# YuliangXiu/ICON

Measured on NVIDIA H100. Metric: M query-points/sec at 256^3 grid, higher is better.
Workload: dtype f32

## Files before the change

icon_b200/_C.py:

```python
import ctypes
import os

_HERE = os.path.dirname(os.path.abspath(__file__))
LIB_PATH = os.environ.get("ICON_B200_LIB") or os.path.join(_HERE, "libicon_b200.so")

if not os.path.exists(LIB_PATH):
    raise ImportError(
        f"{LIB_PATH} is missing: the CUDA extension must be built (python -m icon_b200.build); "
        "icon_b200 has no CPU or PyTorch fallback.")

lib = ctypes.CDLL(LIB_PATH)

_vp, _i, _i64, _f, _sz = ctypes.c_void_p, ctypes.c_int, ctypes.c_int64, ctypes.c_float, ctypes.c_size_t

_SIGS = {
    "icon_version": (_i, []),
    "icon_last_error": (ctypes.c_char_p, []),
    "icon_launch_count": (_i64, []),
    "icon_profile_enable": (_i, [_i]),
    "icon_profile_last_query": (_i, [_vp]),
    "icon_smpl_workspace_bytes": (_sz, [_i, _i]),
    "icon_smpl_prepare": (_i, [_vp, _vp, _vp, _vp, _i, _i, _vp, _sz, _vp]),
    "icon_query_workspace_bytes": (_sz, [_i64, _i, _i]),
    "icon_set_mlp_impl": (_i, [_i]),
    "icon_get_mlp_impl": (_i, []),
    "icon_query": (_i, [_i, _vp, _i64, _i64, _i64, _vp, _vp, _i, _i, _i, _vp, _i, _vp, _i, _i, _vp, _vp, _i, _f,
                        _vp, _vp, _sz, _vp]),
    "icon_query_feats": (_i, [_i, _vp, _i64, _i64, _i64, _vp, _vp, _i, _i, _i, _vp, _i, _vp, _i, _i, _vp, _vp, _i, _f,
                              _i, _vp, _vp, _sz, _vp]),
    "icon_set_sdf_policy": (_i, [_i, _i64, _i64]),
    "icon_set_sdf_bricks": (_i, [_i, _i64]),
    "icon_sdf_brick_info": (_i, [_vp, _i, _i, _vp]),
    "icon_sdf_only": (_i, [_vp, _i64, _i64, _i64, _vp, _vp, _i, _i, _vp, _vp, _vp, _sz, _vp]),
    "icon_sdf_bruteforce": (_i, [_vp, _i64, _i64, _i64, _vp, _vp, _i, _i, _vp, _vp, _vp]),
    "icon_mesh_workspace_bytes": (_sz, [_i, _i]),
    "icon_mesh_prepare": (_i, [_vp, _vp, _i, _i, _vp, _sz, _vp]),
    "icon_mesh_distance": (_i, [_vp, _i64, _vp, _i, _i, _vp, _vp, _vp]),
    "icon_mesh_sample_workspace_bytes": (_sz, [_i]),
    "icon_mesh_sample": (_i, [_vp, _vp, _i, _i, _vp, _i, ctypes.c_uint64, _vp, _vp, _vp, _vp, _sz, _vp]),
    "icon_mlp_only": (_i, [_vp, _i, _i64, _vp, _vp, _vp, _vp]),
    "icon_display": (_i, [_vp, _i, _vp, _vp]),
    "icon_grid_upsample": (_i, [_vp, _vp, _i, _f, _vp, _vp, _vp, _vp]),
    "icon_grid_dilate": (_i, [_vp, _i, _i, _vp, _vp, _vp]),
    "icon_compact_workspace_bytes": (_sz, [_i]),
    "icon_grid_compact": (_i, [_vp, _vp, _i, _i, _vp, _vp, _vp, _vp, _i64, _vp, _vp, _sz, _vp]),
    "icon_grid_scatter": (_i, [_vp, _vp, _vp, _i64, _vp]),
    "icon_grid_init_points": (_i, [_i, _i, _vp, _vp, _vp, _vp]),
    "icon_grid_count_above": (_i, [_vp, _i64, _f, _vp, _vp]),
    "icon_conv_nhwc_workspace_bytes": (_sz, [_i, _i, _i, _i, _i]),
    "icon_conv_nhwc": (_i, [_vp, _vp, _vp, _vp, _vp, _i, _vp, _vp, _vp, _i, _i, _i, _i, _i, _i, _i, _i, _i, _i, _i, _i, _i,
                           _i, _vp, _i, _i, _i, _vp, _vp, _sz, _vp]),
    "icon_norm_finalize": (_i, [_vp, _vp, _vp, _vp, _i, _i, _i, ctypes.c_double, _f, _vp]),
    "icon_act_nhwc": (_i, [_vp, _i, _i, _vp, _vp, _vp, _vp, _i, _f, _vp, _vp, _vp, _vp, _i, _i, _i, _i, _i, _i, _i, _i, _vp]),
    "icon_splitk_instnorm_act": (_i, [_vp, _i, _vp, _vp, _vp, _vp, _vp, _i, _i, _i, _i, _i, _i, _i, _f, _vp]),
    "icon_col2im7": (_i, [_vp, _vp, _vp, _i, _i, _i, _i, _i, _i, _vp]),
    "icon_ew_nhwc": (_i, [_i, _vp, _vp, _vp, _vp, _vp, _i, _i, _i, _i, _vp]),
    "icon_nchw_to_nhwc": (_i, [_vp, _vp, _vp, _i, _i, _i64, _vp]),
    "icon_nhwc_to_nchw": (_i, [_vp, _vp, _i, _i, _i, _i, _i64, _vp]),
# ... 107 lines not shown
```

icon_b200/build.py:

```python
import os
import subprocess
import sys
from concurrent.futures import ThreadPoolExecutor

HERE = os.path.dirname(os.path.abspath(__file__))
CSRC = os.path.join(HERE, "csrc")
OBJ = os.path.join(HERE, "build")
LIB = os.path.join(HERE, "libicon_b200.so")

ARCH = ["-gencode", "arch=compute_90a,code=sm_90a"]
COMMON = ["-O3", "-std=c++17", "-lineinfo", "-Xcompiler", "-fPIC", "-Xcompiler", "-Wall",
          "--expt-relaxed-constexpr"]
SOURCES = {
    "common.cu": [],
    "smpl.cu": ["-fmad=false"],
    "sdf.cu": ["-fmad=false"],
    "mlp.cu": [],
    "mlp_tc.cu": [],
    "engine.cu": [],
    "conv.cu": [],
    "conv_nhwc.cu": [],
    "act_nhwc.cu": [],
    "mc.cu": [],
    "clean.cu": [],
# ... 19 lines not shown
    return out


def gen_tables():
    from . import mc_tables as T
    path = os.path.join(CSRC, "mc_tables.inc")
    lines = ["// GENERATED by icon_b200/build.py from icon_b200/mc_tables.py -- do not edit.",
             "__constant__ unsigned char c_num_verts[256] = {" + ",".join(str(v) for v in T.NUM_VERTS) + "};",
             "__constant__ signed char c_tri_table[256][16] = {"]
    for row in T.TRI_TABLE:
        lines.append("  {" + ",".join(str(v) for v in row) + "},")
    lines.append("};")
    lines.append("__constant__ signed char c_edge_owner[12][4] = {")
    for row in _edge_owner():
        lines.append("  {" + ",".join(str(v) for v in row) + "},")
    lines.append("};")
    text = "\n".join(lines) + "\n"
    if not os.path.exists(path) or open(path).read() != text:
        with open(path, "w") as f:
            f.write(text)
    return path


def _newest_header():
    t = 0.0
    for root, _, files in os.walk(CSRC):
        for f in files:
            if f.endswith((".cuh", ".inc", ".h")):
                t = max(t, os.path.getmtime(os.path.join(root, f)))
    t = max(t, os.path.getmtime(os.path.join(os.path.dirname(HERE), "include", "icon_b200.h")))
    return t


def build(force=False, verbose=False):
    os.makedirs(OBJ, exist_ok=True)
    gen_tables()
    hdr_t = _newest_header()
    jobs = []
    for src, extra in SOURCES.items():
        s = os.path.join(CSRC, src)
        o = os.path.join(OBJ, src.replace(".cu", ".o"))
        if force or not os.path.exists(o) or os.path.getmtime(o) < max(os.path.getmtime(s), hdr_t):
            cmd = ["nvcc", "-c", s, "-o", o] + ARCH + COMMON + extra
            if verbose:
                cmd += ["-Xptxas", "-v"]
            jobs.append(cmd)

    def run(cmd):
        r = subprocess.run(cmd, stdout=subprocess.PIPE, stderr=subprocess.STDOUT, text=True)
        return cmd, r.returncode, r.stdout

    with ThreadPoolExecutor(max_workers=6) as ex:
        for cmd, rc, out in ex.map(run, jobs):
            if verbose or rc:
                print(" ".join(cmd))
                print(out)
            if rc:
                raise RuntimeError("nvcc failed for " + cmd[2])
    objs = [os.path.join(OBJ, s.replace(".cu", ".o")) for s in SOURCES]
    if jobs or force or not os.path.exists(LIB):
        cmd = ["nvcc", "-shared", "-o", LIB] + objs + ARCH + ["-lcudart"]
        subprocess.check_call(cmd)
    return LIB


if __name__ == "__main__":
    print(build(force="--force" in sys.argv, verbose="--verbose" in sys.argv))
```

icon_b200/csrc/mlp_tc.cu:

```cuda
#include <cuda_fp16.h>

#include "common.cuh"
#include "query_common.cuh"
#include "wgmma.cuh"

namespace icon {

constexpr int TC_THREADS = 384;
constexpr int TC_M = 128;
constexpr int NSTAGE = 4;
constexpr int STAGE_BYTES = 32768;
constexpr int STAGES_PER_TILE = 20;
static_assert(STAGES_PER_TILE % NSTAGE == 0 && NSTAGE % 2 == 0, "layer-1 hi / lo pairs must stay on stages (2i, 2i + 1)");
constexpr int GATHER_THREADS = 96;

constexpr int TCB_W0 = 0;
constexpr int TCB_W1 = 32768;
constexpr int TCB_W2 = TCB_W1 + 8 * 65536;
constexpr int TCB_W2T = TCB_W2 + 4 * 32768;
constexpr int TCB_F32 = TCB_W2T + 8192;
constexpr int TCB_F32_FLOATS = 512 + 256 + 128 + 144 + 4;
constexpr int TCB_BYTES = TCB_F32 + TCB_F32_FLOATS * 4;
static_assert(TCB_BYTES == ICON_MLP_TC_BYTES, "blob layout");

constexpr int SM_STAGE = 0;
constexpr int SM_W0 = NSTAGE * STAGE_BYTES;
constexpr int SM_X0 = SM_W0 + 32768;
constexpr int X0_H = 0;
constexpr int X0_L = 4096;
constexpr int X0_F = 8192;
constexpr int X0_SLOT = 16384;
constexpr int SM_F32 = SM_X0 + 2 * X0_SLOT;
constexpr int SM_W2T = (SM_F32 + TCB_F32_FLOATS * 4 + 127) / 128 * 128;
constexpr int SM_BAR = SM_W2T + 8192;
constexpr int NBAR = 2 * NSTAGE + 5;
constexpr int SM_TOTAL = SM_BAR + NBAR * 8;
constexpr int TC_SMEM_BYTES = SM_TOTAL + 1024;
static_assert(TC_SMEM_BYTES <= 227 * 1024, "shared memory");

enum { B_FULL0 = 0, B_EMPTY0 = NSTAGE, B_W0RDY = 2 * NSTAGE, B_XFULL0 = 2 * NSTAGE + 1, B_XEMPTY0 = 2 * NSTAGE + 3 };

constexpr int REG_CONSUMER = 224, REG_PRODUCER = 56;
static_assert(2 * 128 * REG_CONSUMER + 128 * REG_PRODUCER <= 168 * TC_THREADS, "register split");

__device__ __forceinline__ void act_frag64(const float *d, const float *bias, uint32_t (&ah)[4][4], uint32_t (&al)[4][4]) {
#pragma unroll
    for (int kk = 0; kk < 4; ++kk) {
// ... 56 lines not shown
                        if (ch < d) xf[ch * TC_M] = bilinear(q.feat + (size_t)(fb + ch) * q.H * q.W, q.H, q.W, xyz.x, xyz.y);
                }
            } else if (MODE == 1) {
                if (q.C == 12) {
#pragma unroll
                    for (int ch = 0; ch < 12; ++ch)
                        xf[ch * TC_M] = bilinear(q.feat + (size_t)ch * q.H * q.W, q.H, q.W, xyz.x, xyz.y);
                } else {
#pragma unroll
                    for (int ch = 0; ch < 14; ++ch)
                        if (ch < q.C) xf[ch * TC_M] = bilinear(q.feat + (size_t)ch * q.H * q.W, q.H, q.W, xyz.x, xyz.y);
                }
                if (q.C < 15) xf[q.C * TC_M] = xyz.z;
            } else {
                const size_t vs = (size_t)q.VD * q.VD * q.VD;
                if (q.C == 6) {
#pragma unroll
                    for (int ch = 0; ch < 6; ++ch)
                        xf[ch * TC_M] = bilinear(q.feat + (size_t)ch * q.H * q.W, q.H, q.W, xyz.x, xyz.y);
                } else {
#pragma unroll
                    for (int ch = 0; ch < 8; ++ch)
                        if (ch < q.C) xf[ch * TC_M] = bilinear(q.feat + (size_t)ch * q.H * q.W, q.H, q.W, xyz.x, xyz.y);
                }
#pragma unroll
                for (int ch = 0; ch < 7; ++ch)
                    if (q.C + ch < 15) xf[(q.C + ch) * TC_M] = trilinear(q.vol + ch * vs, q.VD, xyz.x, xyz.y, xyz.z);
            }
        }
    }
    xf[15 * TC_M] = in_cube;
}

template <int MODE>
__global__ void __launch_bounds__(TC_THREADS, 1) k_query_mlp_tc(QueryParams q, const uint8_t *__restrict__ blob) {
    using namespace wg;
    extern __shared__ uint8_t smem_raw[];
    const uint32_t raw = s32(smem_raw);
    const uint32_t base = (raw + 1023u) & ~1023u;
    uint8_t *sm = smem_raw + (base - raw);
    const float *sf32 = reinterpret_cast<const float *>(sm + SM_F32);
    const float *sb1 = sf32 + 512, *sw3 = sf32 + 896, *sb3 = sf32 + 1040;
    const uint32_t bar0 = base + SM_BAR;
    auto BAR = [&](int i) { return bar0 + 8u * (uint32_t)i; };

    const int tid = threadIdx.x, warp = tid >> 5, lane = tid & 31;
    const int64_t ntiles = (q.N + TC_M - 1) / TC_M;

    if (tid == 0) {
        for (int s = 0; s < NSTAGE; ++s) { mbar_init(BAR(B_FULL0 + s), 1); mbar_init(BAR(B_EMPTY0 + s), 8); }
        mbar_init(BAR(B_W0RDY), 1);
        for (int b = 0; b < 2; ++b) { mbar_init(BAR(B_XFULL0 + b), GATHER_THREADS); mbar_init(BAR(B_XEMPTY0 + b), 8); }
        asm volatile("fence.mbarrier_init.release.cluster;" ::: "memory");
    }
    __syncthreads();

    if (warp >= 8) {
        asm volatile("setmaxnreg.dec.sync.aligned.u32 %0;" ::"n"(REG_PRODUCER));
        if (warp == 8) {
            if (lane == 0) {
                mbar_expect_tx(BAR(B_W0RDY), 32768 + TCB_F32_FLOATS * 4 + 8192);
                bulk_g2s(base + SM_W0, blob + TCB_W0, 32768, BAR(B_W0RDY));
                bulk_g2s(base + SM_F32, blob + TCB_F32, TCB_F32_FLOATS * 4, BAR(B_W0RDY));
                bulk_g2s(base + SM_W2T, blob + TCB_W2T, 8192, BAR(B_W0RDY));
                uint32_t cnt = 0;
                for (int64_t tile = blockIdx.x; tile < ntiles; tile += gridDim.x) {
                    for (int i = 0; i < STAGES_PER_TILE; ++i, ++cnt) {
                        const uint32_t s = cnt % NSTAGE, ph = (cnt / NSTAGE) & 1;
                        mbar_wait(BAR(B_EMPTY0 + s), ph ^ 1);
                        const uint32_t dst = base + SM_STAGE + s * STAGE_BYTES, full = BAR(B_FULL0 + s);
                        mbar_expect_tx(full, STAGE_BYTES);
                        const uint8_t *src = i < 16 ? blob + TCB_W1 + (size_t)i * 32768 : blob + TCB_W2 + (size_t)(i - 16) * 32768;
                        bulk_g2s(dst, src, STAGE_BYTES, full);
                    }
                }
            }
        } else {
            const int gt = tid - 9 * 32;
            for (uint32_t it = 0; blockIdx.x + (int64_t)it * gridDim.x < ntiles; ++it) {
                const int b = it & 1;
                mbar_wait(BAR(B_XEMPTY0 + b), ((it >> 1) & 1) ^ 1);
                uint8_t *xs = sm + SM_X0 + b * X0_SLOT;
                for (int r = gt; r < TC_M; r += GATHER_THREADS) {
                    float *xf = reinterpret_cast<float *>(xs + X0_F) + r;
                    gather_point<MODE>(q, (blockIdx.x + (int64_t)it * gridDim.x) * TC_M + r, xf);
                    uint32_t hi[8], lo[8];
#pragma unroll
                    for (int i = 0; i < 7; ++i) split2(xf[2 * i * TC_M], xf[(2 * i + 1) * TC_M], hi[i], lo[i]);
                    split2(xf[14 * TC_M], 1.f, hi[7], lo[7]);
                    const int off = (r >> 3) * 128 + (r & 7) * 16;
                    *reinterpret_cast<uint4 *>(xs + X0_H + off) = make_uint4(hi[0], hi[1], hi[2], hi[3]);
                    *reinterpret_cast<uint4 *>(xs + X0_H + off + 2048) = make_uint4(hi[4], hi[5], hi[6], hi[7]);
                    *reinterpret_cast<uint4 *>(xs + X0_L + off) = make_uint4(lo[0], lo[1], lo[2], lo[3]);
                    *reinterpret_cast<uint4 *>(xs + X0_L + off + 2048) = make_uint4(lo[4], lo[5], lo[6], lo[7]);
                }
                fence_proxy_async();
                mbar_arrive(BAR(B_XFULL0 + b));
            }
        }
        return;
    }

    asm volatile("setmaxnreg.inc.sync.aligned.u32 %0;" ::"n"(REG_CONSUMER));
    const int g = warp >> 2;
    const int rf = 64 * g + 16 * (warp & 3) + (lane >> 2);
    const int cq = 2 * (lane & 3);
    uint32_t cnt = 0;
    auto stage_wait = [&](uint32_t c) {
        const uint32_t s = c % NSTAGE;
        mbar_wait(BAR(B_FULL0 + s), (c / NSTAGE) & 1);
        return s;
    };
    auto warp_arrive = [&](int bar) {
        __syncwarp();
        if (lane == 0) mbar_arrive(BAR(bar));
    };
    const uint64_t dw2th = desc_nosw(base + SM_W2T, 2048, 128), dw2tl = desc_nosw(base + SM_W2T + 4096, 2048, 128);
    mbar_wait(BAR(B_W0RDY), 0);

    uint32_t it = 0;
    for (int64_t tile = blockIdx.x; tile < ntiles; tile += gridDim.x, ++it) {
        const int b = it & 1;
        const uint32_t xs = base + SM_X0 + b * X0_SLOT;
        const uint64_t dx0h = desc_nosw(xs + X0_H + g * 1024, 2048, 128), dx0l = desc_nosw(xs + X0_L + g * 1024, 2048, 128);
        mbar_wait(BAR(B_XFULL0 + b), (it >> 1) & 1);

        auto layer0 = [&](int j, float (&a0)[32]) {
            const uint64_t w0h = desc_nosw(base + SM_W0 + j * 1024, 8192, 128), w0l = w0h + (16384 >> 4);
            fence();
            mma_ss<64>(a0, dx0h, w0h, 0);
            mma_ss<64>(a0, dx0h, w0l, 1);
            mma_ss<64>(a0, dx0l, w0h, 1);
            commit();
        };
        float acc1[128];
        auto layer1 = [&](int j, uint32_t (&ch)[4][4], uint32_t (&cl)[4][4], uint32_t (&nh)[4][4], uint32_t (&nl)[4][4]) {
            wait<0>();
            if (j) { warp_arrive(B_EMPTY0 + (cnt - 2) % NSTAGE); warp_arrive(B_EMPTY0 + (cnt - 1) % NSTAGE); }
            float a0[32];
            if (j < 7) layer0(j + 1, a0);
            const uint32_t s = stage_wait(cnt);
            stage_wait(cnt + 1);
            const uint64_t bh = desc_sw128(base + SM_STAGE + s * STAGE_BYTES), bl = bh + (STAGE_BYTES >> 4);
            fence();
#pragma unroll
            for (int kk = 0; kk < 4; ++kk) {
                mma_rs<256>(acc1, ch[kk], bh + 2 * kk, (j | kk) != 0);
                mma_rs<256>(acc1, ch[kk], bl + 2 * kk, 1);
                mma_rs<256>(acc1, cl[kk], bh + 2 * kk, 1);
            }
            commit();
            cnt += 2;
            if (j < 7) {
                wait<1>();
                fence_regs(a0);
                act_frag64(a0, nullptr, nh, nl);
            }
        };
        uint32_t xh[4][4], xl[4][4], yh[4][4], yl[4][4];
        {
            float a0[32];
            layer0(0, a0);
            wait<0>();
            fence_regs(a0);
            act_frag64(a0, nullptr, xh, xl);
        }
#pragma unroll
        for (int j = 0; j < 8; j += 2) {
            layer1(j, xh, xl, yh, yl);
            layer1(j + 1, yh, yl, xh, xl);
        }
        wait<0>();
        fence_regs(acc1);
        warp_arrive(B_EMPTY0 + (cnt - 2) % NSTAGE);
        warp_arrive(B_EMPTY0 + (cnt - 1) % NSTAGE);

        float acc2[64];
        auto layer2 = [&](int c, uint32_t (&ch)[4][4], uint32_t (&cl)[4][4]) {
            const uint32_t s = stage_wait(cnt);
            const uint64_t bh = desc_sw128(base + SM_STAGE + s * STAGE_BYTES), bl = bh + (16384 >> 4);
            fence();
#pragma unroll
            for (int kk = 0; kk < 4; ++kk) {
                mma_rs<128>(acc2, ch[kk], bh + 2 * kk, (c | kk) != 0);
                mma_rs<128>(acc2, ch[kk], bl + 2 * kk, 1);
                mma_rs<128>(acc2, cl[kk], bh + 2 * kk, 1);
            }
            commit();
            ++cnt;
            if (c) {
                wait<1>();
                warp_arrive(B_EMPTY0 + (cnt - 2) % NSTAGE);
            }
        };
        act_frag64(acc1, sb1 + cq, xh, xl);
        layer2(0, xh, xl);
        act_frag64(acc1 + 32, sb1 + 64 + cq, yh, yl);
        layer2(1, yh, yl);
        act_frag64(acc1 + 64, sb1 + 128 + cq, xh, xl);
        layer2(2, xh, xl);
        act_frag64(acc1 + 96, sb1 + 192 + cq, yh, yl);
        layer2(3, yh, yl);
        fence();
        mma_ss<128>(acc2, dx0h, dw2th, 1);
        mma_ss<128>(acc2, dx0h, dw2tl, 1);
        mma_ss<128>(acc2, dx0l, dw2th, 1);
        commit();
        wait<0>();
        fence_regs(acc2);
        warp_arrive(B_EMPTY0 + (cnt - 1) % NSTAGE);

        const float *x0f = reinterpret_cast<const float *>(sm + (xs - base) + X0_F);
        float s0 = 0.f, s1 = 0.f;
#pragma unroll
        for (int i = 0; i < 16; ++i) {
            const float w0 = sw3[8 * i + cq], w1 = sw3[8 * i + cq + 1];
            float v0 = acc2[4 * i], v1 = acc2[4 * i + 1], v2 = acc2[4 * i + 2], v3 = acc2[4 * i + 3];
            v0 = fmaxf(v0, 0.01f * v0); v1 = fmaxf(v1, 0.01f * v1);
            v2 = fmaxf(v2, 0.01f * v2); v3 = fmaxf(v3, 0.01f * v3);
            s0 = fmaf(w0, v0, s0); s0 = fmaf(w1, v1, s0);
            s1 = fmaf(w0, v2, s1); s1 = fmaf(w1, v3, s1);
        }
        s0 += __shfl_xor_sync(0xffffffffu, s0, 1); s0 += __shfl_xor_sync(0xffffffffu, s0, 2);
        s1 += __shfl_xor_sync(0xffffffffu, s1, 1); s1 += __shfl_xor_sync(0xffffffffu, s1, 2);
        if ((lane & 3) < 2) {
            const int r = rf + 8 * (lane & 1);
            float s = (lane & 1) ? s1 : s0;
            const int64_t pi = tile * TC_M + r;
            if (pi < q.N) {
#pragma unroll
                for (int j = 0; j < 15; ++j) s = fmaf(sw3[128 + j], x0f[j * TC_M + r], s);
                s += sb3[0];
                q.out[pi] = x0f[15 * TC_M + r] != 0.f ? s : copysignf(0.f, s);
            }
        }
        warp_arrive(B_XEMPTY0 + b);
    }
}

template <int MODE>
int launch_mlp_tc_t(const QueryParams &q, const void *blob, cudaStream_t stream) {
    static bool attr_set[ICON_MAX_DEVICES] = {};
    if (device_needs_setup(attr_set)) {
        ICON_CUDA(cudaFuncSetAttribute(k_query_mlp_tc<MODE>, cudaFuncAttributeMaxDynamicSharedMemorySize, TC_SMEM_BYTES));
    }

    const int sms = device_sm_count();
    const int64_t ntiles = (q.N + TC_M - 1) / TC_M;
    const unsigned grid = (unsigned)(ntiles < sms ? ntiles : sms);
    k_query_mlp_tc<MODE><<<grid, TC_THREADS, TC_SMEM_BYTES, stream>>>(q, (const uint8_t *)blob);
    ICON_LAUNCHED();
    return ICON_OK;
}

int launch_mlp_tc(int mode, const QueryParams &q, const void *blob, cudaStream_t stream) {
    switch (mode) {
        case 0: return launch_mlp_tc_t<0>(q, blob, stream);
        case 1: return launch_mlp_tc_t<1>(q, blob, stream);
        case 2: return launch_mlp_tc_t<2>(q, blob, stream);
        default: return launch_mlp_tc_t<3>(q, blob, stream);
    }
}

}
```

icon_b200/csrc/wgmma.cuh:

```cuda
#pragma once
#include <cuda.h>
#include <cuda_fp16.h>
#include <stdint.h>

namespace icon {
namespace wg {

__device__ __forceinline__ uint32_t s32(const void *p) { return (uint32_t)__cvta_generic_to_shared(p); }

__device__ __forceinline__ void mbar_init(uint32_t bar, uint32_t count) {
    asm volatile("mbarrier.init.shared::cta.b64 [%0], %1;" ::"r"(bar), "r"(count));
}
__device__ __forceinline__ void mbar_arrive(uint32_t bar) {
    asm volatile("{\n.reg .b64 st;\nmbarrier.arrive.shared::cta.b64 st, [%0];\n}" ::"r"(bar) : "memory");
}
__device__ __forceinline__ void mbar_expect_tx(uint32_t bar, uint32_t bytes) {
    asm volatile("{\n.reg .b64 st;\nmbarrier.arrive.expect_tx.shared::cta.b64 st, [%0], %1;\n}" ::"r"(bar), "r"(bytes) : "memory");
}
__device__ __forceinline__ void mbar_wait(uint32_t bar, uint32_t parity) {
    uint32_t done = 0, spins = 0;
    while (true) {
        asm volatile("{\n.reg .pred q;\nmbarrier.try_wait.parity.shared::cta.b64 q, [%1], %2;\nselp.b32 %0, 1, 0, q;\n}"
                     : "=r"(done) : "r"(bar), "r"(parity) : "memory");
        if (done) break;
        if (++spins > (1u << 24)) __trap();
    }
}
__device__ __forceinline__ void bulk_g2s(uint32_t dst, const void *src, uint32_t bytes, uint32_t bar) {
    asm volatile("cp.async.bulk.shared::cluster.global.mbarrier::complete_tx::bytes [%0], [%1], %2, [%3];" ::"r"(dst),
                 "l"(src), "r"(bytes), "r"(bar) : "memory");
}
__device__ __forceinline__ void tma_load_4d(uint32_t dst, const CUtensorMap *map, int c0, int c1, int c2, int c3,
                                            uint32_t bar) {
    asm volatile("cp.async.bulk.tensor.4d.shared::cluster.global.mbarrier::complete_tx::bytes [%0], [%1, {%3, %4, %5, %6}], [%2];"
                 ::"r"(dst), "l"(reinterpret_cast<uint64_t>(map)), "r"(bar), "r"(c0), "r"(c1), "r"(c2), "r"(c3) : "memory");
}
__device__ __forceinline__ void tma_prefetch_desc(const CUtensorMap *map) {
    asm volatile("prefetch.tensormap [%0];" ::"l"(reinterpret_cast<uint64_t>(map)) : "memory");
}
__device__ __forceinline__ void fence_proxy_async() { asm volatile("fence.proxy.async.shared::cta;" ::: "memory"); }
__device__ __forceinline__ void bar_sync(int id, int threads) { asm volatile("bar.sync %0, %1;" ::"r"(id), "r"(threads) : "memory"); }

__device__ __forceinline__ uint64_t desc_sw128(uint32_t saddr) {
    return (uint64_t)((saddr >> 4) & 0x3FFF) | ((uint64_t)1 << 16) | ((uint64_t)(1024 >> 4) << 32) | ((uint64_t)1 << 62);
}
__device__ __forceinline__ uint64_t desc_nosw(uint32_t saddr, uint32_t lbo, uint32_t sbo) {
    return (uint64_t)((saddr >> 4) & 0x3FFF) | ((uint64_t)((lbo >> 4) & 0x3FFF) << 16) | ((uint64_t)((sbo >> 4) & 0x3FFF) << 32);
}

__device__ __forceinline__ void fence() { asm volatile("wgmma.fence.sync.aligned;" ::: "memory"); }
__device__ __forceinline__ void commit() { asm volatile("wgmma.commit_group.sync.aligned;" ::: "memory"); }
template <int N> __device__ __forceinline__ void wait() { asm volatile("wgmma.wait_group.sync.aligned %0;" ::"n"(N) : "memory"); }
template <int R> __device__ __forceinline__ void fence_regs(float (&d)[R]) {
#pragma unroll
    for (int i = 0; i < R; ++i) asm volatile("" : "+f"(d[i])::"memory");
}

template <int N> __device__ __forceinline__ void mma_ss(float (&d)[N / 2], uint64_t a, uint64_t b, int acc);
template <int N> __device__ __forceinline__ void mma_rs(float (&d)[N / 2], const uint32_t (&a)[4], uint64_t b, int acc);

template <> __device__ __forceinline__ void mma_ss<64>(float (&d)[32], uint64_t a, uint64_t b, int acc) {
    asm volatile("{\n.reg .pred p;\nsetp.ne.b32 p, %34, 0;\n"
                 "wgmma.mma_async.sync.aligned.m64n64k16.f32.f16.f16 {%0,%1,%2,%3,%4,%5,%6,%7,%8,%9,%10,%11,%12,%13,%14,%15,%16,%17,%18,%19,%20,%21,%22,%23,%24,%25,%26,%27,%28,%29,%30,%31}, %32, %33, p, 1, 1, 0, 0;\n}"
                 : "+f"(d[0]), "+f"(d[1]), "+f"(d[2]), "+f"(d[3]), "+f"(d[4]), "+f"(d[5]), "+f"(d[6]), "+f"(d[7]), "+f"(d[8]), "+f"(d[9]), "+f"(d[10]), "+f"(d[11]), "+f"(d[12]), "+f"(d[13]), "+f"(d[14]), "+f"(d[15]), "+f"(d[16]), "+f"(d[17]), "+f"(d[18]), "+f"(d[19]), "+f"(d[20]), "+f"(d[21]), "+f"(d[22]), "+f"(d[23]), "+f"(d[24]), "+f"(d[25]), "+f"(d[26]), "+f"(d[27]), "+f"(d[28]), "+f"(d[29]), "+f"(d[30]), "+f"(d[31])
// ... 38 lines not shown
```

icon_b200/ops.py:

```python
import ctypes

import torch

from . import _C
from ._C import check, lib

PRIOR_ID = {"icon": 0, "pifu": 1, "pamir": 2}
MLP_PACKED_FLOATS = 16 * 512 + 512 + 512 * 256 + 256 + 272 * 128 + 128 + 144 + 1


def _stream():
    return ctypes.c_void_p(torch.cuda.current_stream().cuda_stream)


def _p(t):
    return ctypes.c_void_p(t.data_ptr()) if t is not None else ctypes.c_void_p(0)


def _need_cuda(*ts):
    for t in ts:
        if t is not None and not t.is_cuda:
            raise _C.IconError("icon_b200 ops need CUDA tensors: there is no CPU path")


# ... 104 lines not shown
    rows, K = M.shape
    src = M.reshape(rows // 8, 8, K // 8, 8)
    return np.ascontiguousarray(src.transpose(2, 0, 1, 3)).tobytes()


def pack_mlp(sd, c0, prefix="", device=None):
    import numpy as np
    (W0, W1, W2, W3), (b0, b1, b2, b3) = _fold_mlp(sd, c0, prefix)
    f32 = torch.cat([W0.t().contiguous().reshape(-1), b0, W1.t().contiguous().reshape(-1), b1,
                     W2.t().contiguous().reshape(-1), b2, W3, b3]).float()
    assert f32.numel() == MLP_PACKED_FLOATS
    blob = bytearray()
    W0b = W0.clone(); W0b[:, 15] = b0
    W2b = W2.clone(); W2b[:, 256 + 15] = b2
    h, l = _hi_lo(W0b)
    blob += _img_nosw(h) + _img_nosw(l)
    h, l = _hi_lo(W1)
    for j in range(8):
        blob += _img_sw128(h[:, 64 * j:64 * j + 64]) + _img_sw128(l[:, 64 * j:64 * j + 64])
    h, l = _hi_lo(W2b)
    for j in range(4):
        blob += _img_sw128(h[:, 64 * j:64 * j + 64]) + _img_sw128(l[:, 64 * j:64 * j + 64])
    blob += _img_nosw(np.ascontiguousarray(h[:, 256:272])) + _img_nosw(np.ascontiguousarray(l[:, 256:272]))
    tail = torch.cat([b0, b1, b2, W3, b3, torch.zeros(3)]).float().numpy().tobytes()
    blob += tail
    assert len(blob) == MLP_TC_BYTES, (len(blob), MLP_TC_BYTES)
    tc = torch.frombuffer(blob, dtype=torch.uint8).clone()
    out = PackedMLP(f32, tc, c0)
    return out.to(device) if device is not None else out


def set_mlp_impl(name):
    check(lib.icon_set_mlp_impl({"fp32": 0, "tcgen05": 1}[name]), "icon_set_mlp_impl")


def set_sdf_policy(force_ppw=0, ppw8_from=-1, ppw32_from=-1):
    check(lib.icon_set_sdf_policy(int(force_ppw), int(ppw8_from), int(ppw32_from)), "icon_set_sdf_policy")


def set_sdf_bricks(enable=True, max_entries=0):
    check(lib.icon_set_sdf_bricks(int(bool(enable)), int(max_entries)), "icon_set_sdf_bricks")


def sdf_brick_info(body):
    out = (ctypes.c_int64 * 5)()
    check(lib.icon_sdf_brick_info(_p(body.ws), body.V, body.F, out), "icon_sdf_brick_info")
    return dict(zip(("built", "overflow", "entries", "capacity", "builds"), (int(v) for v in out)))


def _point_strides(points):
    if points.dim() != 3 or points.shape[0] != 1 or points.shape[1] != 3:
        raise _C.IconError(f"points must be [1,3,N], got {tuple(points.shape)}")
    if points.dtype != torch.float32:
        points = points.float()
    return points, points.stride(1), points.stride(2), points.shape[2]


SMPL_FEATS_ALL = ("sdf", "cmap", "norm", "vis")
FEAT_CMAP, FEAT_NORM, FEAT_VIS = 1, 2, 4
_FEAT_BIT = {"sdf": 0, "cmap": FEAT_CMAP, "norm": FEAT_NORM, "vis": FEAT_VIS}


def smpl_feats_mask(smpl_feats):
    unknown = set(smpl_feats) - set(_FEAT_BIT)
    if unknown:
        raise _C.IconError(f"smpl_feats: unknown feature(s) {sorted(unknown)}; the icon prior knows {list(SMPL_FEATS_ALL)}")
# ... 198 lines not shown
```

include/icon_b200.h:

```cpp
#ifndef ICON_B200_H
#define ICON_B200_H

#include <stddef.h>
#include <stdint.h>

#ifdef __cplusplus
extern "C" {
#endif

#define ICON_OK 0
#define ICON_EINVAL (-1)
#define ICON_ECUDA (-2)
#define ICON_ENOSPC (-3)

#define ICON_PRIOR_ICON 0
#define ICON_PRIOR_PIFU 1
#define ICON_PRIOR_PAMIR 2

typedef void *icon_stream_t;

int icon_version(void);
const char *icon_last_error(void);
int64_t icon_launch_count(void);

int icon_profile_enable(int on);
int icon_profile_last_query(float *h_ms);

size_t icon_smpl_workspace_bytes(int V, int F);
int icon_smpl_prepare(const float *verts, const int64_t *faces, const float *cmap,
                      const float *vis, int V, int F, void *mesh_ws, size_t mesh_ws_bytes,
                      icon_stream_t stream);

#define ICON_MLP_PACKED_FLOATS (16 * 512 + 512 + 512 * 256 + 256 + 272 * 128 + 128 + 144 + 1)
#define ICON_MLP_TC_BYTES (32768 + 8 * 65536 + 4 * 32768 + 8192 + (512 + 256 + 128 + 144 + 4) * 4)
int icon_set_mlp_impl(int impl);
int icon_get_mlp_impl(void);

size_t icon_query_workspace_bytes(int64_t N, int F, int prior);
int icon_query(int prior, const float *points, int64_t stride_c, int64_t stride_n, int64_t N,
               const float *h_calib, const float *feat, int C, int H, int W,
               const float *vol_feat, int VD, const void *mesh_ws, int V, int F,
               const float *mlp_packed, const void *mlp_tc, int c0, float sdf_clip, float *out,
               void *ws, size_t ws_bytes, icon_stream_t stream);

#define ICON_FEAT_CMAP 1
#define ICON_FEAT_NORM 2
#define ICON_FEAT_VIS 4
#define ICON_FEAT_ALL (ICON_FEAT_CMAP | ICON_FEAT_NORM | ICON_FEAT_VIS)
int icon_query_feats(int prior, const float *points, int64_t stride_c, int64_t stride_n, int64_t N,
                     const float *h_calib, const float *feat, int C, int H, int W,
                     const float *vol_feat, int VD, const void *mesh_ws, int V, int F,
                     const float *mlp_packed, const void *mlp_tc, int c0, float sdf_clip, int smpl_feats,
                     float *out, void *ws, size_t ws_bytes, icon_stream_t stream);

int icon_set_sdf_policy(int force_ppw, int64_t ppw8_from, int64_t ppw32_from);
int icon_set_sdf_bricks(int enable, int64_t max_entries);
int icon_sdf_brick_info(const void *mesh_ws, int V, int F, int64_t *out);

int icon_sdf_only(const float *points, int64_t stride_c, int64_t stride_n, int64_t N,
                  const float *h_calib, const void *mesh_ws, int V, int F, float *rec,
                  int32_t *face, void *ws, size_t ws_bytes, icon_stream_t stream);
int icon_sdf_bruteforce(const float *points, int64_t stride_c, int64_t stride_n, int64_t N,
                        const float *h_calib, const void *mesh_ws, int V, int F, float *rec,
                        int32_t *face, icon_stream_t stream);
size_t icon_mesh_workspace_bytes(int V, int F);
int icon_mesh_prepare(const float *verts, const int64_t *faces, int V, int F, void *mesh_ws, size_t mesh_ws_bytes,
                      icon_stream_t stream);
int icon_mesh_distance(const float *points, int64_t N, const void *mesh_ws, int V, int F, float *out_sqdist,
                       int32_t *out_face, icon_stream_t stream);
// ... 228 lines not shown
```

Before: 543.6.

## Multicast MLP weight stages across 2-CTA clusters in tensor-core query kernel

Launches the wgmma MLP kernel as 2-CTA clusters, with each CTA loading half of every weight stage via TMA multicast into both CTAs' shared memory. Consumers release stages to every CTA in the cluster through cluster-mapped mbarriers, and the producer drains the pipeline before exit. The aim is to halve L2-to-SM weight traffic, which is streamed per tile. In exchange the paired CTAs must run in lockstep, the grid is sized by cluster occupancy, and optional clock-based stats instrumentation plus a build helper for defines are added.

```diff
diff --git a/icon_b200/_C.py b/icon_b200/_C.py
--- a/icon_b200/_C.py
+++ b/icon_b200/_C.py
@@ -24,6 +24,7 @@
     "icon_query_workspace_bytes": (_sz, [_i64, _i, _i]),
     "icon_set_mlp_impl": (_i, [_i]),
     "icon_get_mlp_impl": (_i, []),
+    "icon_set_mlp_cluster": (_i, [_i]),
     "icon_query": (_i, [_i, _vp, _i64, _i64, _i64, _vp, _vp, _i, _i, _i, _vp, _i, _vp, _i, _i, _vp, _vp, _i, _f,
                         _vp, _vp, _sz, _vp]),
     "icon_query_feats": (_i, [_i, _vp, _i64, _i64, _i64, _vp, _vp, _i, _i, _i, _vp, _i, _vp, _i, _i, _vp, _vp, _i, _f,
diff --git a/icon_b200/build.py b/icon_b200/build.py
--- a/icon_b200/build.py
+++ b/icon_b200/build.py
@@ -75,16 +75,18 @@
     return t
 
 
-def build(force=False, verbose=False):
-    os.makedirs(OBJ, exist_ok=True)
+def build(force=False, verbose=False, out_dir=None, defines=()):
+    obj_dir = os.path.join(out_dir, "build") if out_dir else OBJ
+    lib = os.path.join(out_dir, "libicon_b200.so") if out_dir else LIB
+    os.makedirs(obj_dir, exist_ok=True)
     gen_tables()
     hdr_t = _newest_header()
     jobs = []
     for src, extra in SOURCES.items():
         s = os.path.join(CSRC, src)
-        o = os.path.join(OBJ, src.replace(".cu", ".o"))
+        o = os.path.join(obj_dir, src.replace(".cu", ".o"))
         if force or not os.path.exists(o) or os.path.getmtime(o) < max(os.path.getmtime(s), hdr_t):
-            cmd = ["nvcc", "-c", s, "-o", o] + ARCH + COMMON + extra
+            cmd = ["nvcc", "-c", s, "-o", o] + ARCH + COMMON + extra + ["-D" + d for d in defines]
             if verbose:
                 cmd += ["-Xptxas", "-v"]
             jobs.append(cmd)
@@ -100,11 +102,11 @@
                 print(out)
             if rc:
                 raise RuntimeError("nvcc failed for " + cmd[2])
-    objs = [os.path.join(OBJ, s.replace(".cu", ".o")) for s in SOURCES]
-    if jobs or force or not os.path.exists(LIB):
-        cmd = ["nvcc", "-shared", "-o", LIB] + objs + ARCH + ["-lcudart"]
+    objs = [os.path.join(obj_dir, s.replace(".cu", ".o")) for s in SOURCES]
+    if jobs or force or not os.path.exists(lib):
+        cmd = ["nvcc", "-shared", "-o", lib] + objs + ARCH + ["-lcudart"]
         subprocess.check_call(cmd)
-    return LIB
+    return lib
 
 
 if __name__ == "__main__":
diff --git a/icon_b200/csrc/mlp_tc.cu b/icon_b200/csrc/mlp_tc.cu
--- a/icon_b200/csrc/mlp_tc.cu
+++ b/icon_b200/csrc/mlp_tc.cu
@@ -13,6 +13,7 @@
 constexpr int STAGES_PER_TILE = 20;
 static_assert(STAGES_PER_TILE % NSTAGE == 0 && NSTAGE % 2 == 0, "layer-1 hi / lo pairs must stay on stages (2i, 2i + 1)");
 constexpr int GATHER_THREADS = 96;
+constexpr int MLP_CLUSTER = 2;
 
 constexpr int TCB_W0 = 0;
 constexpr int TCB_W1 = 32768;
@@ -135,7 +136,20 @@
     xf[15 * TC_M] = in_cube;
 }
 
-template <int MODE>
+#ifdef ICON_MLP_STATS
+constexpr int MLP_STATS_CTAS = 1024;
+__device__ unsigned long long g_mlp_stats[MLP_STATS_CTAS][8];
+#define MLP_TIMED(acc, stmt) do { const long long t_ = clock64(); stmt; acc += clock64() - t_; } while (0)
+__device__ __forceinline__ unsigned long long globaltimer() {
+    unsigned long long t;
+    asm volatile("mov.u64 %0, %%globaltimer;" : "=l"(t));
+    return t;
+}
+#else
+#define MLP_TIMED(acc, stmt) stmt
+#endif
+
+template <int MODE, int CL>
 __global__ void __launch_bounds__(TC_THREADS, 1) k_query_mlp_tc(QueryParams q, const uint8_t *__restrict__ blob) {
     using namespace wg;
     extern __shared__ uint8_t smem_raw[];
@@ -149,14 +163,20 @@
 
     const int tid = threadIdx.x, warp = tid >> 5, lane = tid & 31;
     const int64_t ntiles = (q.N + TC_M - 1) / TC_M;
+#ifdef ICON_MLP_STATS
+    long long t_wait = 0;
+    const long long t_start = clock64();
+    const unsigned long long ns_start = globaltimer();
+#endif
 
     if (tid == 0) {
-        for (int s = 0; s < NSTAGE; ++s) { mbar_init(BAR(B_FULL0 + s), 1); mbar_init(BAR(B_EMPTY0 + s), 8); }
+        for (int s = 0; s < NSTAGE; ++s) { mbar_init(BAR(B_FULL0 + s), 1); mbar_init(BAR(B_EMPTY0 + s), 8 * CL); }
         mbar_init(BAR(B_W0RDY), 1);
         for (int b = 0; b < 2; ++b) { mbar_init(BAR(B_XFULL0 + b), GATHER_THREADS); mbar_init(BAR(B_XEMPTY0 + b), 8); }
         asm volatile("fence.mbarrier_init.release.cluster;" ::: "memory");
     }
-    __syncthreads();
+    if (CL == 1) __syncthreads();
+    else cluster_sync();
 
     if (warp >= 8) {
         asm volatile("setmaxnreg.dec.sync.aligned.u32 %0;" ::"n"(REG_PRODUCER));
@@ -167,20 +187,31 @@
                 bulk_g2s(base + SM_F32, blob + TCB_F32, TCB_F32_FLOATS * 4, BAR(B_W0RDY));
                 bulk_g2s(base + SM_W2T, blob + TCB_W2T, 8192, BAR(B_W0RDY));
                 uint32_t cnt = 0;
-                for (int64_t tile = blockIdx.x; tile < ntiles; tile += gridDim.x) {
+                for (int64_t tile = blockIdx.x; tile - blockIdx.x % CL < ntiles; tile += gridDim.x) {
                     for (int i = 0; i < STAGES_PER_TILE; ++i, ++cnt) {
                         const uint32_t s = cnt % NSTAGE, ph = (cnt / NSTAGE) & 1;
-                        mbar_wait(BAR(B_EMPTY0 + s), ph ^ 1);
+                        MLP_TIMED(t_wait, mbar_wait(BAR(B_EMPTY0 + s), ph ^ 1));
                         const uint32_t dst = base + SM_STAGE + s * STAGE_BYTES, full = BAR(B_FULL0 + s);
                         mbar_expect_tx(full, STAGE_BYTES);
                         const uint8_t *src = i < 16 ? blob + TCB_W1 + (size_t)i * 32768 : blob + TCB_W2 + (size_t)(i - 16) * 32768;
-                        bulk_g2s(dst, src, STAGE_BYTES, full);
+                        if (CL == 1) {
+                            bulk_g2s(dst, src, STAGE_BYTES, full);
+                        } else {
+                            constexpr uint32_t PART = STAGE_BYTES / CL;
+                            const uint32_t rank = blockIdx.x % CL;
+                            bulk_g2s_multicast(dst + rank * PART, src + rank * PART, PART, full, (uint16_t)((1u << CL) - 1));
+                        }
                     }
                 }
+                for (int i = 0; CL > 1 && i < NSTAGE; ++i, ++cnt)
+                    mbar_wait(BAR(B_EMPTY0 + cnt % NSTAGE), ((cnt / NSTAGE) & 1) ^ 1);
+#ifdef ICON_MLP_STATS
+                if (blockIdx.x < MLP_STATS_CTAS) g_mlp_stats[blockIdx.x][3] = t_wait;
+#endif
             }
         } else {
             const int gt = tid - 9 * 32;
-            for (uint32_t it = 0; blockIdx.x + (int64_t)it * gridDim.x < ntiles; ++it) {
+            for (uint32_t it = 0; blockIdx.x - blockIdx.x % CL + it * gridDim.x < (uint32_t)ntiles; ++it) {
                 const int b = it & 1;
                 mbar_wait(BAR(B_XEMPTY0 + b), ((it >> 1) & 1) ^ 1);
                 uint8_t *xs = sm + SM_X0 + b * X0_SLOT;
@@ -209,24 +240,35 @@
     const int rf = 64 * g + 16 * (warp & 3) + (lane >> 2);
     const int cq = 2 * (lane & 3);
     uint32_t cnt = 0;
+#ifdef ICON_MLP_STATS
+    long long t_xwait = 0;
+#endif
     auto stage_wait = [&](uint32_t c) {
         const uint32_t s = c % NSTAGE;
-        mbar_wait(BAR(B_FULL0 + s), (c / NSTAGE) & 1);
+        MLP_TIMED(t_wait, mbar_wait(BAR(B_FULL0 + s), (c / NSTAGE) & 1));
         return s;
     };
     auto warp_arrive = [&](int bar) {
         __syncwarp();
         if (lane == 0) mbar_arrive(BAR(bar));
     };
+    auto release_stage = [&](uint32_t s) {
+        if (CL == 1) {
+            warp_arrive(B_EMPTY0 + s);
+        } else {
+            __syncwarp();
+            if (lane < CL) mbar_arrive_cluster(mapa(BAR(B_EMPTY0 + s), lane));
+        }
+    };
     const uint64_t dw2th = desc_nosw(base + SM_W2T, 2048, 128), dw2tl = desc_nosw(base + SM_W2T + 4096, 2048, 128);
     mbar_wait(BAR(B_W0RDY), 0);
 
     uint32_t it = 0;
-    for (int64_t tile = blockIdx.x; tile < ntiles; tile += gridDim.x, ++it) {
+    for (int64_t tile = blockIdx.x; tile - blockIdx.x % CL < ntiles; tile += gridDim.x, ++it) {
         const int b = it & 1;
         const uint32_t xs = base + SM_X0 + b * X0_SLOT;
         const uint64_t dx0h = desc_nosw(xs + X0_H + g * 1024, 2048, 128), dx0l = desc_nosw(xs + X0_L + g * 1024, 2048, 128);
-        mbar_wait(BAR(B_XFULL0 + b), (it >> 1) & 1);
+        MLP_TIMED(t_xwait, mbar_wait(BAR(B_XFULL0 + b), (it >> 1) & 1));
 
         auto layer0 = [&](int j, float (&a0)[32]) {
             const uint64_t w0h = desc_nosw(base + SM_W0 + j * 1024, 8192, 128), w0l = w0h + (16384 >> 4);
@@ -239,7 +281,7 @@
         float acc1[128];
         auto layer1 = [&](int j, uint32_t (&ch)[4][4], uint32_t (&cl)[4][4], uint32_t (&nh)[4][4], uint32_t (&nl)[4][4]) {
             wait<0>();
-            if (j) { warp_arrive(B_EMPTY0 + (cnt - 2) % NSTAGE); warp_arrive(B_EMPTY0 + (cnt - 1) % NSTAGE); }
+            if (j) { release_stage((cnt - 2) % NSTAGE); release_stage((cnt - 1) % NSTAGE); }
             float a0[32];
             if (j < 7) layer0(j + 1, a0);
             const uint32_t s = stage_wait(cnt);
@@ -275,8 +317,8 @@
         }
         wait<0>();
         fence_regs(acc1);
-        warp_arrive(B_EMPTY0 + (cnt - 2) % NSTAGE);
-        warp_arrive(B_EMPTY0 + (cnt - 1) % NSTAGE);
+        release_stage((cnt - 2) % NSTAGE);
+        release_stage((cnt - 1) % NSTAGE);
 
         float acc2[64];
         auto layer2 = [&](int c, uint32_t (&ch)[4][4], uint32_t (&cl)[4][4]) {
@@ -293,7 +335,7 @@
             ++cnt;
             if (c) {
                 wait<1>();
-                warp_arrive(B_EMPTY0 + (cnt - 2) % NSTAGE);
+                release_stage((cnt - 2) % NSTAGE);
             }
         };
         act_frag64(acc1, sb1 + cq, xh, xl);
@@ -311,7 +353,7 @@
         commit();
         wait<0>();
         fence_regs(acc2);
-        warp_arrive(B_EMPTY0 + (cnt - 1) % NSTAGE);
+        release_stage((cnt - 1) % NSTAGE);
 
         const float *x0f = reinterpret_cast<const float *>(sm + (xs - base) + X0_F);
         float s0 = 0.f, s1 = 0.f;
@@ -339,30 +381,81 @@
         }
         warp_arrive(B_XEMPTY0 + b);
     }
-}
-
-template <int MODE>
+#ifdef ICON_MLP_STATS
+    if (lane == 0 && blockIdx.x < MLP_STATS_CTAS) {
+        unsigned long long *st = g_mlp_stats[blockIdx.x];
+        atomicAdd(st + 1, (unsigned long long)t_wait);
+        atomicAdd(st + 2, (unsigned long long)t_xwait);
+        if (warp == 0) {
+            unsigned smid;
+            asm volatile("mov.u32 %0, %%smid;" : "=r"(smid));
+            st[0] = clock64() - t_start; st[4] = it; st[5] = ns_start; st[6] = globaltimer(); st[7] = smid;
+        }
+    }
+#endif
+}
+
+static int g_mlp_cluster = MLP_CLUSTER;
+
+template <int MODE, int CL>
 int launch_mlp_tc_t(const QueryParams &q, const void *blob, cudaStream_t stream) {
     static bool attr_set[ICON_MAX_DEVICES] = {};
-    if (device_needs_setup(attr_set)) {
-        ICON_CUDA(cudaFuncSetAttribute(k_query_mlp_tc<MODE>, cudaFuncAttributeMaxDynamicSharedMemorySize, TC_SMEM_BYTES));
-    }
-
-    const int sms = device_sm_count();
-    const int64_t ntiles = (q.N + TC_M - 1) / TC_M;
-    const unsigned grid = (unsigned)(ntiles < sms ? ntiles : sms);
-    k_query_mlp_tc<MODE><<<grid, TC_THREADS, TC_SMEM_BYTES, stream>>>(q, (const uint8_t *)blob);
+    static int max_clusters[ICON_MAX_DEVICES] = {};
+    cudaLaunchConfig_t cfg = {};
+    cudaLaunchAttribute attr[1];
+    attr[0].id = cudaLaunchAttributeClusterDimension;
+    attr[0].val.clusterDim.x = CL; attr[0].val.clusterDim.y = 1; attr[0].val.clusterDim.z = 1;
+    cfg.blockDim = dim3(TC_THREADS); cfg.dynamicSmemBytes = TC_SMEM_BYTES; cfg.stream = stream;
+    cfg.attrs = attr; cfg.numAttrs = CL > 1 ? 1 : 0;
+    int dev = 0;
+    if (device_needs_setup(attr_set, &dev)) {
+        ICON_CUDA(cudaFuncSetAttribute(k_query_mlp_tc<MODE, CL>, cudaFuncAttributeMaxDynamicSharedMemorySize, TC_SMEM_BYTES));
+        int n = device_sm_count() / CL;
+        if (CL > 1) {
+            cfg.gridDim = dim3(CL * n);
+            ICON_CUDA(cudaOccupancyMaxActiveClusters(&n, k_query_mlp_tc<MODE, CL>, &cfg));
+        }
+        max_clusters[dev] = n;
+    }
+    if (max_clusters[dev] < 1) {
+        set_error("k_query_mlp_tc: no cluster of %d CTAs fits on device %d", CL, dev);
+        return ICON_ECUDA;
+    }
+    const int64_t ngroups = ((q.N + TC_M - 1) / TC_M + CL - 1) / CL;
+    cfg.gridDim = dim3((unsigned)(CL * (ngroups < max_clusters[dev] ? ngroups : max_clusters[dev])));
+    ICON_CUDA(cudaLaunchKernelEx(&cfg, k_query_mlp_tc<MODE, CL>, q, (const uint8_t *)blob));
     ICON_LAUNCHED();
     return ICON_OK;
 }
 
+template <int MODE>
+int launch_mlp_tc_m(const QueryParams &q, const void *blob, cudaStream_t stream) {
+    return g_mlp_cluster == 1 ? launch_mlp_tc_t<MODE, 1>(q, blob, stream) : launch_mlp_tc_t<MODE, MLP_CLUSTER>(q, blob, stream);
+}
+
 int launch_mlp_tc(int mode, const QueryParams &q, const void *blob, cudaStream_t stream) {
     switch (mode) {
-        case 0: return launch_mlp_tc_t<0>(q, blob, stream);
-        case 1: return launch_mlp_tc_t<1>(q, blob, stream);
-        case 2: return launch_mlp_tc_t<2>(q, blob, stream);
-        default: return launch_mlp_tc_t<3>(q, blob, stream);
-    }
-}
-
-}
+        case 0: return launch_mlp_tc_m<0>(q, blob, stream);
+        case 1: return launch_mlp_tc_m<1>(q, blob, stream);
+        case 2: return launch_mlp_tc_m<2>(q, blob, stream);
+        default: return launch_mlp_tc_m<3>(q, blob, stream);
+    }
+}
+
+}
+
+extern "C" int icon_set_mlp_cluster(int size) {
+    ICON_CHECK_ARG(size == 1 || size == icon::MLP_CLUSTER, "icon_set_mlp_cluster: 1 or %d", icon::MLP_CLUSTER);
+    icon::g_mlp_cluster = size;
+    return ICON_OK;
+}
+
+#ifdef ICON_MLP_STATS
+extern "C" int icon_mlp_stats(unsigned long long *out, int reset) {
+    ICON_CUDA(cudaMemcpyFromSymbol(out, icon::g_mlp_stats, sizeof(icon::g_mlp_stats)));
+    void *p = nullptr;
+    ICON_CUDA(cudaGetSymbolAddress(&p, icon::g_mlp_stats));
+    if (reset) ICON_CUDA(cudaMemset(p, 0, sizeof(icon::g_mlp_stats)));
+    return ICON_OK;
+}
+#endif
diff --git a/icon_b200/csrc/wgmma.cuh b/icon_b200/csrc/wgmma.cuh
--- a/icon_b200/csrc/wgmma.cuh
+++ b/icon_b200/csrc/wgmma.cuh
@@ -30,6 +30,24 @@
     asm volatile("cp.async.bulk.shared::cluster.global.mbarrier::complete_tx::bytes [%0], [%1], %2, [%3];" ::"r"(dst),
                  "l"(src), "r"(bytes), "r"(bar) : "memory");
 }
+__device__ __forceinline__ void bulk_g2s_multicast(uint32_t dst, const void *src, uint32_t bytes, uint32_t bar,
+                                                   uint16_t cta_mask) {
+    asm volatile("cp.async.bulk.shared::cluster.global.mbarrier::complete_tx::bytes.multicast::cluster [%0], [%1], %2, [%3], %4;"
+                 ::"r"(dst), "l"(src), "r"(bytes), "r"(bar), "h"(cta_mask) : "memory");
+}
+
+__device__ __forceinline__ uint32_t mapa(uint32_t saddr, uint32_t rank) {
+    uint32_t r;
+    asm volatile("mapa.shared::cluster.u32 %0, %1, %2;" : "=r"(r) : "r"(saddr), "r"(rank));
+    return r;
+}
+__device__ __forceinline__ void mbar_arrive_cluster(uint32_t cluster_bar) {
+    asm volatile("mbarrier.arrive.shared::cluster.b64 _, [%0];" ::"r"(cluster_bar) : "memory");
+}
+__device__ __forceinline__ void cluster_sync() {
+    asm volatile("barrier.cluster.arrive.release;\nbarrier.cluster.wait.acquire;" ::: "memory");
+}
+
 __device__ __forceinline__ void tma_load_4d(uint32_t dst, const CUtensorMap *map, int c0, int c1, int c2, int c3,
                                             uint32_t bar) {
     asm volatile("cp.async.bulk.tensor.4d.shared::cluster.global.mbarrier::complete_tx::bytes [%0], [%1, {%3, %4, %5, %6}], [%2];"
diff --git a/icon_b200/ops.py b/icon_b200/ops.py
--- a/icon_b200/ops.py
+++ b/icon_b200/ops.py
@@ -160,6 +160,10 @@
 
 def set_mlp_impl(name):
     check(lib.icon_set_mlp_impl({"fp32": 0, "tcgen05": 1}[name]), "icon_set_mlp_impl")
+
+
+def set_mlp_cluster(size):
+    check(lib.icon_set_mlp_cluster(int(size)), "icon_set_mlp_cluster")
 
 
 def set_sdf_policy(force_ppw=0, ppw8_from=-1, ppw32_from=-1):
diff --git a/include/icon_b200.h b/include/icon_b200.h
--- a/include/icon_b200.h
+++ b/include/icon_b200.h
@@ -35,6 +35,7 @@
 #define ICON_MLP_TC_BYTES (32768 + 8 * 65536 + 4 * 32768 + 8192 + (512 + 256 + 128 + 144 + 4) * 4)
 int icon_set_mlp_impl(int impl);
 int icon_get_mlp_impl(void);
+int icon_set_mlp_cluster(int size);
 
 size_t icon_query_workspace_bytes(int64_t N, int F, int prior);
 int icon_query(int prior, const float *points, int64_t stride_c, int64_t stride_n, int64_t N,
```

Result: faster. 553.5 (median of 6 runs) (+1.8%).
